# mauriceqch/pcc_geo_cnn_v2

Measured on AMD Instinct MI355X. Metric: voxel_blocks_64cubed_per_sec_encode_decode, higher is better.
Workload: dtype f32

## Files before the change

pcc_geo_cnn_v2_amd/csrc/conv_tr2m_f16s.hip:

```cpp
#include <cstdlib>

#include "tr2m_common.h"

namespace pcctr2mh {

using namespace pcck;
using namespace pcctr2;

__device__ __forceinline__ u32x4 split_quad(const f32x4& v, const f32x2& s2) {
    f32x2 lo, hi;
    asm("v_pk_mul_f32 %0, %1, %2" : "=v"(lo) : "v"(__builtin_shufflevector(v, v, 0, 1)), "v"(s2));
    asm("v_pk_mul_f32 %0, %1, %2" : "=v"(hi) : "v"(__builtin_shufflevector(v, v, 2, 3)), "v"(s2));
    const unsigned h01 = __builtin_bit_cast(unsigned, __builtin_convertvector(lo, f16x2)), h23 = __builtin_bit_cast(unsigned, __builtin_convertvector(hi, f16x2));
    unsigned l01, l23;
    asm volatile("v_fma_mixlo_f16 %0, %1, -1.0, %2 op_sel:[0,0,0] op_sel_hi:[1,0,0]\n\t"
                 "v_fma_mixhi_f16 %0, %1, -1.0, %3 op_sel:[1,0,0] op_sel_hi:[1,0,0]" : "=&v"(l01) : "v"(h01), "v"(lo[0]), "v"(lo[1]));
    asm volatile("v_fma_mixlo_f16 %0, %1, -1.0, %2 op_sel:[0,0,0] op_sel_hi:[1,0,0]\n\t"
                 "v_fma_mixhi_f16 %0, %1, -1.0, %3 op_sel:[1,0,0] op_sel_hi:[1,0,0]" : "=&v"(l23) : "v"(h23), "v"(hi[0]), "v"(hi[1]));
    return (u32x4){h01, h23, l01, l23};
}
template <int OFF>
__device__ __forceinline__ u32x4 lds_read2_dup(unsigned addr) {
    u32x4 v;
    asm volatile("ds_read2_b64 %0, %1 offset0:%2 offset1:%2" : "=v"(v) : "v"(addr), "n"(OFF / 8));
    return v;
}
template <int N>
__device__ __forceinline__ void lgkm_wait_w(u32x4& a, u32x4& b) { asm volatile("s_waitcnt lgkmcnt(%2)" : "+v"(a), "+v"(b) : "n"(N)); }
__device__ __forceinline__ unsigned tr2m_scale_bits(unsigned m, int lsu) {
    if (m == 0u) return 0x3f800000u;
    int se = 268 - (int)(m >> 23);
    const int lo = 7 - lsu > 1 ? 7 - lsu : 1, hi = 247 - lsu < 254 ? 247 - lsu : 254;
    se = se < lo ? lo : se > hi ? hi : se;
    return (unsigned)se << 23;
}

constexpr int VSB = 96;
constexpr int TILE_BYTES = ITEMS * 64 * VSB;
constexpr int W_BASE = TILE_BYTES;
constexpr int WL_LANE = 27 * 16 + 8;
constexpr int WG_BYTES = 64 * WL_LANE;
constexpr int ROWB = LXY * VSB;

struct Tr2mArgs {
    const float* in;
    const float* w;
    const float* wtail;
    const unsigned* amax_in;
    const float* bias;
    float* out;
    Tr2mGrid g;
    unsigned* amax_out = nullptr;
};

template <int NG, bool RELU>
__global__ void __launch_bounds__(NT, 1) conv_tr2m_f16s_kernel(Tr2mArgs a, int nwg) {
    extern __shared__ __attribute__((aligned(16))) unsigned char smem[];
    const int tid = threadIdx.x, lane = tid & 63, wave = __builtin_amdgcn_readfirstlane(tid >> 6);
    const int v = lane & 15, cq = lane >> 4;
    auto ldsu = [&](unsigned off) -> u32x4 { return *reinterpret_cast<const u32x4*>(smem + off); };
    typedef __attribute__((address_space(3))) void* lds_ptr;

    const Tr2mTile tile = tr2m_tile(a.g, nwg);
    const int ct = tile.ct, n = tile.n, X0 = tile.X0, Y0 = tile.Y0, zb = tile.zb;
    const int nsteps = a.g.zlen + 1;
    constexpr int CIN = NG * 16;
    const size_t HW = (size_t)a.g.H * a.g.W;
    const unsigned HWI = (unsigned)(HW * CIN * 4);
    const float* in_n = a.in + (size_t)n * a.g.D * HW * CIN;

    {
        constexpr int WBYTES = NG * WG_BYTES, NCH = (WBYTES + 1023) / 1024;
        const __amdgpu_buffer_rsrc_t rw = make_rsrc(a.w + (size_t)ct * (WBYTES / 4), (unsigned)WBYTES);
        for (int p = wave; p < NCH; p += 4)
            __builtin_amdgcn_raw_ptr_buffer_load_lds(rw, (lds_ptr)(smem + W_BASE + p * 1024), 16, lane * 16, p * 1024, 0, 0);
    }
    const float su = a.wtail[0];
    const unsigned sbits = tr2m_scale_bits(pcc_amax_read(a.amax_in + (size_t)n * PCC_AMAX_SLOTS), (int)(__builtin_bit_cast(unsigned, su) >> 23) - 127);
    const float sv = __builtin_bit_cast(float, sbits);
    const float sprod = su * sv, sinv = 1.0f / sprod;
    const f32x2 sc2 = {sv, sv}, inv2 = {sinv, sinv};
    const int gperm = ((tid >> 2) & ~3) | (((tid >> 2) & 1) << 1) | (((tid >> 2) >> 1) & 1);
    unsigned rel[ITEMS];
#pragma unroll
    for (int it = 0; it < ITEMS; ++it) {
        const int item = it * NT + tid;
        const int u = it * 64 + gperm, q = item & 3, ly = u / LXY, lx = u - ly * LXY;
        const int y = Y0 - 1 + ly, x = X0 - 1 + lx;
        const bool ok = item < TILE_SLOTS && y >= 0 && y < a.g.H && x >= 0 && x < a.g.W;
        rel[it] = ok ? (unsigned)(((y * a.g.W + x) * CIN + q * 4) * 4) : kOOB;
    }
    const unsigned cw = (unsigned)(gperm * VSB + (tid & 3) * 16);
    f32x4 stg[ITEMS];
    auto fetch_tile = [&](int sp, int cg, unsigned long long addr) __attribute__((always_inline)) {
        const bool ok = (unsigned)(zb - 1 + sp) < (unsigned)a.g.D && sp < nsteps;
        const __amdgpu_buffer_rsrc_t rp = make_rsrc((const void*)(ok ? addr : (unsigned long long)in_n), ok ? HWI - (unsigned)(64 * cg) : 0u);
#pragma unroll
        for (int it = 0; it < ITEMS; ++it) stg[it] = __builtin_bit_cast(f32x4, __builtin_amdgcn_raw_buffer_load_b128(rp, (int)rel[it], 0, 0));
    };
    auto commit2 = [&](auto j_tag) __attribute__((always_inline)) {
        constexpr int j = decltype(j_tag)::value, j1 = j + 1 < ITEMS ? j + 1 : j;
        *reinterpret_cast<u32x4*>(smem + cw + (unsigned)(j * 64 * VSB)) = split_quad(stg[j], sc2);
        if constexpr (j1 != j) *reinterpret_cast<u32x4*>(smem + cw + (unsigned)(j1 * 64 * VSB)) = split_quad(stg[j1], sc2);
    };

    unsigned ba[2];
#pragma unroll
    for (int dxi = 0; dxi < 2; ++dxi) ba[dxi] = (unsigned)((4 * wave * LXY + v + 1 - dxi) * VSB + cq * 16);
    unsigned wa = (unsigned)(unsigned long long)(lds_ptr)smem + (unsigned)(W_BASE + lane * WL_LANE);

    const int OH = 2 * a.g.H, OW = 2 * a.g.W;
    const unsigned ob = (unsigned)((((2 * (Y0 + 4 * wave)) * OW + 2 * (X0 + v)) * a.g.ocs + a.g.oco + 16 * ct + 4 * cq) * 4);
    const unsigned PLANE_O = (unsigned)((size_t)OH * OW * a.g.ocs * 4);
    float* out_n = a.out + (size_t)n * (2 * a.g.D) * OH * OW * a.g.ocs;
    const f32x4 zero4 = {0.f, 0.f, 0.f, 0.f};
    f32x4 bias_l = (a.g.flags & PCC_CONV_BIAS) ? *reinterpret_cast<const f32x4*>(a.bias + 16 * ct + 4 * cq) : zero4;
#pragma unroll
    for (int cc = 0; cc < 4; ++cc) bias_l[cc] *= sprod;

    int s2 = 0, c2 = 0;
    unsigned long long tile_pl = (unsigned long long)in_n + (unsigned long long)(long long)(zb - 1) * HWI;
    auto fetch_next = [&]() __attribute__((always_inline)) {
        fetch_tile(s2, c2, tile_pl);
        tr2m_next_tile<NG, 64>(s2, c2, tile_pl, HWI);
    };
    fetch_next();
    commit2(std::integral_constant<int, 0>{}); commit2(std::integral_constant<int, 2>{}); commit2(std::integral_constant<int, 4>{});
    fetch_next();
    __builtin_amdgcn_s_waitcnt(0x0F70);
    __syncthreads();

    f32x4 E[2][4][4], O[4][4];
    u32x4 b1[2][2][4];
    u32x4 wf1[3], wf2[3];
    auto load_b = [&]() __attribute__((always_inline)) {
#pragma unroll
        for (int dyi = 0; dyi < 2; ++dyi)
#pragma unroll
            for (int dxi = 0; dxi < 2; ++dxi)
#pragma unroll
                for (int i = 0; i < 4; ++i)
                    b1[dyi][dxi][i] = ldsu(ba[dxi] + (unsigned)((i + 1 - dyi) * ROWB));
    };
    auto load_w = [&](auto slot_tag, auto sq_tag) __attribute__((always_inline)) {
        constexpr int slot = decltype(slot_tag)::value, sq = decltype(sq_tag)::value;
        wf2[slot] = lds_read2_dup<sq * 16 + 8>(wa);
        wf1[slot] = lds_read2_dup<sq * 16>(wa);
    };
    using I0 = std::integral_constant<int, 0>;
    using I1 = std::integral_constant<int, 1>;
    load_b();
    load_w(I0{}, std::integral_constant<int, tap_of(18).sq>{}); load_w(I1{}, std::integral_constant<int, tap_of(19).sq>{});

    int s = 0, c = 0;
    unsigned long long out_pl = (unsigned long long)out_n + (unsigned long long)(long long)(2 * (zb - 2)) * PLANE_O;

    float mx = 0.f, mxt = 0.f;
    auto finish = [&](auto ph_tag, auto e_tag, const __amdgpu_buffer_rsrc_t& rout, f32x4& keep) __attribute__((always_inline)) {
        constexpr int PH = decltype(ph_tag)::value, e = decltype(e_tag)::value;
        constexpr int pz = e < 16 ? 1 : 0, cls = (e >> 2) & 3, i = e & 3, py = cls >> 1, px = cls & 1;
        f32x4 o = acc_read(pz ? O[cls][i] : E[PH ^ 1][cls][i]);
        if (RELU) o = __builtin_elementwise_maximum(o, zero4);
        o = mul4s(o, inv2);
        keep = o;
        asm("v_max3_f32 %0, %0, |%1|, |%2|" : "+v"(mxt) : "v"(o[0]), "v"(o[1]));
        asm("v_max3_f32 %0, %0, |%1|, |%2|" : "+v"(mxt) : "v"(o[2]), "v"(o[3]));
        const unsigned soff = (unsigned)pz * PLANE_O + (unsigned)(((2 * i + py) * OW + px) * a.g.ocs * 4);
        buf_store4(rout, keep, ob, soff);
    };

    auto micro = [&](auto ph_tag, auto first_tag, auto halo_tag) __attribute__((always_inline)) {
        constexpr int PH = decltype(ph_tag)::value;
        constexpr bool FIRST = decltype(first_tag)::value, HALO = decltype(halo_tag)::value;
        constexpr int T0 = HALO ? 18 : 0;
        const bool prev_ok = s >= 2;
        const __amdgpu_buffer_rsrc_t rout = make_rsrc((const void*)(prev_ok ? out_pl : (unsigned long long)out_n), FIRST && prev_ok ? 2u * PLANE_O : 0u);
        f32x4 ost[2][3];
        static_for(std::make_integer_sequence<int, 27 - T0>{}, [&](auto t_tag) __attribute__((always_inline)) {
            constexpr int t = decltype(t_tag)::value + T0;
            constexpr Tap T = tap_of(t);
            if constexpr (t + 2 < 27) load_w(std::integral_constant<int, (t + 2 - T0) % 3>{}, std::integral_constant<int, tap_of(t + 2).sq>{});
            lgkm_wait_w<(t + 2 < 27 ? 4 : t + 1 < 27 ? 2 : 0)>(wf1[(t - T0) % 3], wf2[(t - T0) % 3]);
            constexpr bool open = FIRST && T.opens && T.kz != 0;
#pragma unroll
            for (int tm = 0; tm < 2; ++tm)
#pragma unroll
                for (int i = 0; i < 4; ++i) {
                    f32x4& acc = T.kz == 0 ? E[PH][T.cls][i] : T.kz == 1 ? O[T.cls][i] : E[PH ^ 1][T.cls][i];
                    acc = mfma_f16(tm == 1 ? wf2[(t - T0) % 3] : wf1[(t - T0) % 3], b1[T.dyi][T.dxi][i], (open && tm == 0) ? bias_l : acc);
                }
#ifndef PCC_TR2MB_INTERLEAVE
            __builtin_amdgcn_sched_barrier(0);
#endif
            if constexpr (t == T0) __syncthreads();
            if constexpr (t == 26) {
                commit2(std::integral_constant<int, 0>{}); commit2(std::integral_constant<int, 2>{}); commit2(std::integral_constant<int, 4>{});
                fetch_next();
            }
            if constexpr (FIRST && !HALO) tr2m_finish_under_tap<t>(finish, ph_tag, rout, ost);
            __builtin_amdgcn_sched_barrier(0);
        });
        if constexpr (FIRST && !HALO) { mx = fmaxf(mx, prev_ok ? mxt : 0.f); mxt = 0.f; }
        __builtin_amdgcn_s_waitcnt(0xC07F);
        __syncthreads();
        if (++c == NG) { c = 0; ++s; out_pl += 2ull * PLANE_O; wa -= (unsigned)((NG - 1) * WG_BYTES); } else wa += (unsigned)WG_BYTES;
        load_b();
        if (s == 0) { load_w(I0{}, std::integral_constant<int, tap_of(18).sq>{}); load_w(I1{}, std::integral_constant<int, tap_of(19).sq>{}); }
        else { load_w(I0{}, std::integral_constant<int, tap_of(0).sq>{}); load_w(I1{}, std::integral_constant<int, tap_of(1).sq>{}); }
    };
    auto plane = [&](auto ph_tag, auto halo_tag) __attribute__((always_inline)) {
        micro(ph_tag, std::true_type{}, halo_tag);
#pragma unroll
        for (int k = 1; k < NG; ++k) micro(ph_tag, std::false_type{}, halo_tag);
    };
    plane(std::integral_constant<int, 0>{}, std::true_type{});
#pragma nounroll
    for (int sp = 1; sp < nsteps; sp += 2) {
        plane(std::integral_constant<int, 1>{}, std::false_type{});
        if (sp + 1 < nsteps) plane(std::integral_constant<int, 0>{}, std::false_type{});
    }
    {
        const __amdgpu_buffer_rsrc_t rout = make_rsrc((const void*)out_pl, nsteps >= 2 ? 2u * PLANE_O : 0u);
        f32x4 keep[32];
        if (nsteps & 1) tr2m_drain<1>(finish, rout, keep);
        else tr2m_drain<0>(finish, rout, keep);
#pragma unroll
        for (int e = 0; e < 32; ++e) asm volatile("" ::"v"(keep[e]));
        mx = fmaxf(mx, nsteps >= 2 ? mxt : 0.f);
    }
    if (a.amax_out != nullptr) pcc_amax_record(a.amax_out + (size_t)n * PCC_AMAX_SLOTS, mx, (int)blockIdx.x * 4 + wave);
}

}

using namespace pcctr2mh;

size_t pcc_tr2m_f16s_packed_floats(int Cin, int Cout) { return (size_t)(Cout / 16) * (Cin / 16) * (WG_BYTES / 4) + PCC_TR2M_F16S_TAIL; }
void pcc_tr2m_f16s_pack(int Cin, int Cout, const float* w_tr2g, float* out) {
    const int NGi = Cin / 16, NCT = Cout / 16;
    const size_t nfrag = (size_t)NGi * 27 * NCT;
    const float su = f16s_weight_scale(w_tr2g, nfrag * 256);
    memset(out, 0, pcc_tr2m_f16s_packed_floats(Cin, Cout) * sizeof(float));
    unsigned short* o = reinterpret_cast<unsigned short*>(out);
    for (int g = 0; g < NGi; ++g)
        for (int sq = 0; sq < 27; ++sq)
            for (int ct = 0; ct < NCT; ++ct)
                for (int lane = 0; lane < 64; ++lane) {
                    unsigned short* d = o + ((size_t)(ct * NGi + g) * WG_BYTES + (size_t)lane * WL_LANE + (size_t)sq * 16) / 2;
                    for (int c = 0; c < 4; ++c) {
                        const float x = w_tr2g[((((size_t)g * 27 + sq) * NCT + ct) * 64 + lane) * 4 + c] * su;
                        d[c] = f16_bits(x);
                        d[4 + c] = f16_bits(x - f16_value(d[c]));
                    }
                }
    out[(size_t)NCT * NGi * (WG_BYTES / 4)] = su;
}

int pcc_conv_tr2m_f16s(pcc_ctx* ctx, const pcc_conv_desc* d, const float* in, const float* w_f16s, const float* bias, float* out,
                       pcc_conv_ext* ext, hipStream_t st) {
    PCC_REQUIRE(pcc_tr2m_eligible(d), "pcc_conv_tr2m_f16s: shape not covered");
    const int NGi = d->Cin / 16;
    Tr2mArgs a;
    a.in = in; a.w = w_f16s; a.bias = bias; a.out = out;
    a.wtail = w_f16s + (size_t)(d->Cout / 16) * NGi * (WG_BYTES / 4);
    if (ext) ext->out_recorded = false;
    if (ext && ext->out_amax) { a.amax_out = ext->out_amax; ext->out_recorded = true; }
    if (ext && ext->in_amax) a.amax_in = ext->in_amax;
    else {
        unsigned* am = nullptr;
        { const int rc = pcc_ctx_amax(ctx, d->N * PCC_AMAX_SLOTS, &am); if (rc != PCC_OK) return rc; }
        { const int rc = pcc_block_amax(ctx, in, d->N, (size_t)d->D * d->H * d->W * d->Cin, am, st); if (rc != PCC_OK) return rc; }
        a.amax_in = am;
    }
    const int nwg = tr2m_grid(ctx, d, a.g);
    const int lds = W_BASE + ((NGi * WG_BYTES + 1023) / 1024) * 1024;
    typedef void (*kern_t)(Tr2mArgs, int);
    static const kern_t kerns[4] = {conv_tr2m_f16s_kernel<2, false>, conv_tr2m_f16s_kernel<2, true>, conv_tr2m_f16s_kernel<4, false>, conv_tr2m_f16s_kernel<4, true>};
    return tr2m_launch(kerns[(NGi == 4 ? 2 : 0) + ((d->flags & PCC_CONV_RELU) ? 1 : 0)], lds, nwg, a, st);
}
```

Measured before the change: 8553.

## Spread tr2m output stores across first and last micro-steps of each plane

Output plane stores, previously all issued under the first micro-step of each plane, are now split. Part of them are written early during the last micro-step of the previous plane, and the rest during the first micro-step. This spreads store traffic and the finish work more evenly across the MFMA schedule, and the final drain handles only the remaining items. An optional s_memtime probe, off by default, is added to measure barrier and wait costs. The risks are more register pressure from the extra live values and a harder-to-follow store schedule.

```diff
diff --git a/pcc_geo_cnn_v2_amd/csrc/conv_tr2m_f16s.hip b/pcc_geo_cnn_v2_amd/csrc/conv_tr2m_f16s.hip
--- a/pcc_geo_cnn_v2_amd/csrc/conv_tr2m_f16s.hip
+++ b/pcc_geo_cnn_v2_amd/csrc/conv_tr2m_f16s.hip
@@ -1,11 +1,39 @@
 #include <cstdlib>
 
 #include "tr2m_common.h"
+
+#ifndef PCC_TR2M_SPREAD
+#define PCC_TR2M_SPREAD 1
+#endif
+#ifndef PCC_TR2M_PROBE
+#define PCC_TR2M_PROBE 0
+#endif
+#if PCC_TR2M_PROBE
+#include <algorithm>
+#include <cstdio>
+#include <vector>
+#define PCC_TR2M_STAMPED(...) __VA_ARGS__
+#else
+#define PCC_TR2M_STAMPED(...)
+#endif
 
 namespace pcctr2mh {
 
 using namespace pcck;
 using namespace pcctr2;
+
+#if PCC_TR2M_PROBE
+constexpr int PROBE_PLACES = 5;
+constexpr int PROBE_KINDS = 3;
+constexpr int PROBE_WORDS = PROBE_KINDS * PROBE_PLACES + PROBE_KINDS;
+__device__ __forceinline__ unsigned long long tr2m_stamp() {
+    unsigned long long t;
+    __builtin_amdgcn_sched_barrier(0);
+    asm volatile("s_memtime %0\n\ts_waitcnt lgkmcnt(0)" : "=s"(t) :: "memory");
+    __builtin_amdgcn_sched_barrier(0);
+    return t;
+}
+#endif
 
 __device__ __forceinline__ u32x4 split_quad(const f32x4& v, const f32x2& s2) {
     f32x2 lo, hi;
@@ -42,6 +70,20 @@
 constexpr int WG_BYTES = 64 * WL_LANE;
 constexpr int ROWB = LXY * VSB;
 
+constexpr bool f16s_item_is_early(int e) { return e < 16 ? e < 9 : e < 25; }
+template <int t, class F, class PH, class V>
+__device__ __forceinline__ void f16s_finish_early(F& finish, PH ph_next, const __amdgpu_buffer_rsrc_t& rout, V (&ost)[2][3]) {
+    if constexpr (t >= 9 && t < 18) finish(ph_next, std::integral_constant<int, 16 + (t - 9)>{}, rout, ost[t & 1][0]);
+    if constexpr (t >= 18) finish(ph_next, std::integral_constant<int, t - 18>{}, rout, ost[t & 1][0]);
+    if constexpr (t >= 10) asm volatile("" ::"v"(ost[(t - 1) & 1][0]));
+}
+template <int t, class F, class PH, class V>
+__device__ __forceinline__ void f16s_finish_late(F& finish, PH ph_tag, const __amdgpu_buffer_rsrc_t& rout, V (&ost)[2][3]) {
+    if constexpr (t < 7) finish(ph_tag, std::integral_constant<int, 9 + t>{}, rout, ost[t & 1][0]);
+    if constexpr (t >= 9 && t < 16) finish(ph_tag, std::integral_constant<int, 16 + t>{}, rout, ost[t & 1][0]);
+    if constexpr ((t >= 1 && t < 8) || (t >= 10 && t < 17)) asm volatile("" ::"v"(ost[(t - 1) & 1][0]));
+}
+
 struct Tr2mArgs {
     const float* in;
     const float* w;
@@ -51,6 +93,7 @@
     float* out;
     Tr2mGrid g;
     unsigned* amax_out = nullptr;
+    PCC_TR2M_STAMPED(unsigned* stamps = nullptr;)
 };
 
 template <int NG, bool RELU>
@@ -149,6 +192,7 @@
     };
     using I0 = std::integral_constant<int, 0>;
     using I1 = std::integral_constant<int, 1>;
+    PCC_TR2M_STAMPED(unsigned pacc[PROBE_KINDS][PROBE_PLACES] = {}; unsigned pcnt[PROBE_KINDS] = {}; unsigned long long pt_end = tr2m_stamp();)
     load_b();
     load_w(I0{}, std::integral_constant<int, tap_of(18).sq>{}); load_w(I1{}, std::integral_constant<int, tap_of(19).sq>{});
 
@@ -169,18 +213,23 @@
         buf_store4(rout, keep, ob, soff);
     };
 
-    auto micro = [&](auto ph_tag, auto first_tag, auto halo_tag) __attribute__((always_inline)) {
+    auto micro = [&](auto ph_tag, auto first_tag, auto halo_tag, auto last_tag) __attribute__((always_inline)) {
         constexpr int PH = decltype(ph_tag)::value;
-        constexpr bool FIRST = decltype(first_tag)::value, HALO = decltype(halo_tag)::value;
+        constexpr bool FIRST = decltype(first_tag)::value, HALO = decltype(halo_tag)::value, LASTM = decltype(last_tag)::value;
         constexpr int T0 = HALO ? 18 : 0;
+        constexpr bool STORES = FIRST && !HALO;
+        constexpr bool EARLY = LASTM && !HALO && PCC_TR2M_SPREAD;
+        PCC_TR2M_STAMPED(constexpr int pk = HALO ? 2 : FIRST ? 0 : 1; unsigned long long pa = 0;)
         const bool prev_ok = s >= 2;
-        const __amdgpu_buffer_rsrc_t rout = make_rsrc((const void*)(prev_ok ? out_pl : (unsigned long long)out_n), FIRST && prev_ok ? 2u * PLANE_O : 0u);
+        const __amdgpu_buffer_rsrc_t rout = EARLY ? make_rsrc((const void*)(out_pl + 2ull * PLANE_O), 2u * PLANE_O)
+                                                  : make_rsrc((const void*)(prev_ok ? out_pl : (unsigned long long)out_n), FIRST && prev_ok ? 2u * PLANE_O : 0u);
         f32x4 ost[2][3];
         static_for(std::make_integer_sequence<int, 27 - T0>{}, [&](auto t_tag) __attribute__((always_inline)) {
             constexpr int t = decltype(t_tag)::value + T0;
             constexpr Tap T = tap_of(t);
             if constexpr (t + 2 < 27) load_w(std::integral_constant<int, (t + 2 - T0) % 3>{}, std::integral_constant<int, tap_of(t + 2).sq>{});
             lgkm_wait_w<(t + 2 < 27 ? 4 : t + 1 < 27 ? 2 : 0)>(wf1[(t - T0) % 3], wf2[(t - T0) % 3]);
+            PCC_TR2M_STAMPED(if constexpr (t == T0) pacc[pk][0] += (unsigned)(tr2m_stamp() - pt_end);)
             constexpr bool open = FIRST && T.opens && T.kz != 0;
 #pragma unroll
             for (int tm = 0; tm < 2; ++tm)
@@ -192,26 +241,41 @@
 #ifndef PCC_TR2MB_INTERLEAVE
             __builtin_amdgcn_sched_barrier(0);
 #endif
+            PCC_TR2M_STAMPED(if constexpr (t == T0) pa = tr2m_stamp();)
             if constexpr (t == T0) __syncthreads();
+            PCC_TR2M_STAMPED(if constexpr (t == T0) pacc[pk][1] += (unsigned)(tr2m_stamp() - pa);)
             if constexpr (t == 26) {
+                PCC_TR2M_STAMPED(
+                    pa = tr2m_stamp();
+                    _Pragma("unroll") for (int it = 0; it < ITEMS; ++it) asm volatile("" : "+v"(stg[it]));
+                    pacc[pk][2] += (unsigned)(tr2m_stamp() - pa);)
                 commit2(std::integral_constant<int, 0>{}); commit2(std::integral_constant<int, 2>{}); commit2(std::integral_constant<int, 4>{});
                 fetch_next();
             }
-            if constexpr (FIRST && !HALO) tr2m_finish_under_tap<t>(finish, ph_tag, rout, ost);
+            if constexpr (STORES && !PCC_TR2M_SPREAD) tr2m_finish_under_tap<t>(finish, ph_tag, rout, ost);
+            if constexpr (STORES && PCC_TR2M_SPREAD) f16s_finish_late<t>(finish, ph_tag, rout, ost);
+            if constexpr (EARLY) f16s_finish_early<t>(finish, std::integral_constant<int, PH ^ 1>{}, rout, ost);
             __builtin_amdgcn_sched_barrier(0);
         });
+        if constexpr (EARLY) asm volatile("" ::"v"(ost[0][0]));
         if constexpr (FIRST && !HALO) { mx = fmaxf(mx, prev_ok ? mxt : 0.f); mxt = 0.f; }
+        PCC_TR2M_STAMPED(pa = tr2m_stamp();)
         __builtin_amdgcn_s_waitcnt(0xC07F);
         __syncthreads();
+        PCC_TR2M_STAMPED({ const unsigned long long pb = tr2m_stamp(); pacc[pk][3] += (unsigned)(pb - pa); pacc[pk][4] += (unsigned)(pb - pt_end); pt_end = pb; ++pcnt[pk]; })
         if (++c == NG) { c = 0; ++s; out_pl += 2ull * PLANE_O; wa -= (unsigned)((NG - 1) * WG_BYTES); } else wa += (unsigned)WG_BYTES;
         load_b();
         if (s == 0) { load_w(I0{}, std::integral_constant<int, tap_of(18).sq>{}); load_w(I1{}, std::integral_constant<int, tap_of(19).sq>{}); }
         else { load_w(I0{}, std::integral_constant<int, tap_of(0).sq>{}); load_w(I1{}, std::integral_constant<int, tap_of(1).sq>{}); }
     };
     auto plane = [&](auto ph_tag, auto halo_tag) __attribute__((always_inline)) {
-        micro(ph_tag, std::true_type{}, halo_tag);
-#pragma unroll
-        for (int k = 1; k < NG; ++k) micro(ph_tag, std::false_type{}, halo_tag);
+        static_assert(NG == 2 || NG == 4, "the plane is written out");
+        micro(ph_tag, std::true_type{}, halo_tag, std::false_type{});
+        if constexpr (NG == 4) {
+            micro(ph_tag, std::false_type{}, halo_tag, std::false_type{});
+            micro(ph_tag, std::false_type{}, halo_tag, std::false_type{});
+        }
+        micro(ph_tag, std::false_type{}, halo_tag, std::true_type{});
     };
     plane(std::integral_constant<int, 0>{}, std::true_type{});
 #pragma nounroll
@@ -222,13 +286,34 @@
     {
         const __amdgpu_buffer_rsrc_t rout = make_rsrc((const void*)out_pl, nsteps >= 2 ? 2u * PLANE_O : 0u);
         f32x4 keep[32];
+#if PCC_TR2M_SPREAD
+        auto rest = [&](auto ph_tag) __attribute__((always_inline)) {
+            static_for(std::make_integer_sequence<int, 32>{}, [&](auto e_tag) __attribute__((always_inline)) {
+                if constexpr (!f16s_item_is_early(decltype(e_tag)::value)) finish(ph_tag, e_tag, rout, keep[decltype(e_tag)::value]); });
+        };
+        if (nsteps & 1) rest(std::integral_constant<int, 1>{});
+        else rest(std::integral_constant<int, 0>{});
+#else
         if (nsteps & 1) tr2m_drain<1>(finish, rout, keep);
         else tr2m_drain<0>(finish, rout, keep);
-#pragma unroll
-        for (int e = 0; e < 32; ++e) asm volatile("" ::"v"(keep[e]));
+#endif
+#pragma unroll
+        for (int e = 0; e < 32; ++e)
+            if (!PCC_TR2M_SPREAD || !f16s_item_is_early(e)) asm volatile("" ::"v"(keep[e]));
         mx = fmaxf(mx, nsteps >= 2 ? mxt : 0.f);
     }
     if (a.amax_out != nullptr) pcc_amax_record(a.amax_out + (size_t)n * PCC_AMAX_SLOTS, mx, (int)blockIdx.x * 4 + wave);
+#if PCC_TR2M_PROBE
+    if (a.stamps != nullptr && lane == 0) {
+        unsigned* p = a.stamps + ((size_t)blockIdx.x * 4 + wave) * PROBE_WORDS;
+#pragma unroll
+        for (int k = 0; k < PROBE_KINDS; ++k) {
+#pragma unroll
+            for (int j = 0; j < PROBE_PLACES; ++j) p[k * PROBE_PLACES + j] = pacc[k][j];
+            p[PROBE_KINDS * PROBE_PLACES + k] = pcnt[k];
+        }
+    }
+#endif
 }
 
 }
@@ -276,5 +361,44 @@
     const int lds = W_BASE + ((NGi * WG_BYTES + 1023) / 1024) * 1024;
     typedef void (*kern_t)(Tr2mArgs, int);
     static const kern_t kerns[4] = {conv_tr2m_f16s_kernel<2, false>, conv_tr2m_f16s_kernel<2, true>, conv_tr2m_f16s_kernel<4, false>, conv_tr2m_f16s_kernel<4, true>};
+#if PCC_TR2M_PROBE
+    {
+        static unsigned* dev = nullptr;
+        static size_t cap = 0;
+        const size_t words = (size_t)nwg * 4 * PROBE_WORDS;
+        if (words > cap) {
+            if (dev) PCC_CHECK_HIP(hipFree(dev));
+            dev = nullptr; cap = 0;
+            PCC_CHECK_HIP(hipMalloc((void**)&dev, words * sizeof(unsigned)));
+            cap = words;
+        }
+        PCC_CHECK_HIP(hipMemsetAsync(dev, 0, words * sizeof(unsigned), st));
+        a.stamps = dev;
+        const int rc = tr2m_launch(kerns[(NGi == 4 ? 2 : 0) + ((d->flags & PCC_CONV_RELU) ? 1 : 0)], lds, nwg, a, st);
+        if (rc != PCC_OK) return rc;
+        std::vector<unsigned> h(words);
+        PCC_CHECK_HIP(hipMemcpyAsync(h.data(), dev, words * sizeof(unsigned), hipMemcpyDeviceToHost, st));
+        PCC_CHECK_HIP(hipStreamSynchronize(st));
+        static const char* kinds[PROBE_KINDS] = {"first", "other", "halo"};
+        for (int k = 0; k < PROBE_KINDS; ++k) {
+            double med[PROBE_PLACES];
+            size_t waves = 0;
+            for (int j = 0; j < PROBE_PLACES; ++j) {
+                std::vector<double> v;
+                for (size_t w = 0; w < (size_t)nwg * 4; ++w) {
+                    const unsigned* p = h.data() + w * PROBE_WORDS;
+                    if (p[PROBE_KINDS * PROBE_PLACES + k]) v.push_back((double)p[k * PROBE_PLACES + j] / p[PROBE_KINDS * PROBE_PLACES + k]);
+                }
+                waves = v.size();
+                std::sort(v.begin(), v.end());
+                med[j] = v.empty() ? 0.0 : v[v.size() / 2];
+            }
+            fprintf(stderr, "tr2m_probe spread=%d NG=%d nwg=%d zlen=%d kind=%s waves=%zu first_tap=%.0f barrier_T0=%.0f vmcnt_wait=%.0f closing_barrier=%.0f micro_step=%.0f\n",
+                    PCC_TR2M_SPREAD, NGi, nwg, a.g.zlen, kinds[k], waves, med[0], med[1], med[2], med[3], med[4]);
+        }
+        return PCC_OK;
+    }
+#else
     return tr2m_launch(kerns[(NGi == 4 ? 2 : 0) + ((d->flags & PCC_CONV_RELU) ? 1 : 0)], lds, nwg, a, st);
-}
+#endif
+}
```

Result: slower. 8200 (-4.1%).
